# georgeyounes/CRIMP

Measured on AMD Instinct MI355X. Metric: Z^2_2 photon*trial evals/sec (node), higher is better.
Workload: dtype f64; 1 GPU; config3: synthetic 10000000 photons x 1000000 trials/GPU, Z^2_2; photons=10000000, trials_per_gpu=1000000, nharm=2, parallelism=trial-sharded dp1: sharding.sharded_search + all_gather(best), precision=default

## Files before the change

crimp_amd/csrc/search_nufft.h:

```cpp
#pragma once

typedef double nu_f64x4 __attribute__((ext_vector_type(4)));

constexpr int kNuCW = 1024;
constexpr int kNuWaves = 4;
constexpr int kNuRows = 8;
constexpr int kNuMaxP = 16;
constexpr int kNuGatherMaxP = 24;
constexpr int kNuMergeG = 16;
constexpr int kNuMaxWrap = 32;
constexpr int kNuTile = 4096;
constexpr double kNuEps = 5e-14;
constexpr double kNuEpsZm = 5e-13;
constexpr double kNuRho = 1e-13;

constexpr int kNuPassMax = 10;
struct NuPass {
    int64_t gmin[kNuPassMax];
    int64_t ubase[kNuPassMax];
};

struct NuTw {
    const double2* lo;
    const double2* hi;
// ... 429 lines not shown
        }
    }
    for (int o = L / 2; o > 0; o >>= 1)
#pragma unroll
        for (int r = 0; r < R; ++r)
#pragma unroll
            for (int p = 0; p < PP; ++p)
                if (p < P) {
                    ar[r][p] += __shfl_xor(ar[r][p], o);
                    ai[r][p] += __shfl_xor(ai[r][p], o);
                }
#pragma unroll
    for (int r = 0; r < R; ++r)
#pragma unroll
        for (int p = 0; p < PP; ++p)
            if (r < nrow && p < P && (p & (L - 1)) == sub)
                W[((int64_t)p * nrow + r) * nfft + g] = make_double2(ar[r][p], ai[r][p]);
}

__global__ __launch_bounds__(256) void k_nu_merge(const double* __restrict__ U, int64_t SL,
                                                  const int64_t* __restrict__ ctab, int64_t nchunk, int64_t gmin,
                                                  int64_t gmax, int64_t nfft, int64_t gbase, int64_t gcount,
                                                  double2* __restrict__ W, const int* __restrict__ bad) {
    if (*bad) return;
    __shared__ int64_t rs[kNuMergeG][kNuMaxWrap];
    __shared__ int rc[kNuMergeG][kNuMaxWrap];
    __shared__ int nr[kNuMergeG];
    extern __shared__ double nu_acc[];
    const int64_t i0 = (int64_t)blockIdx.x * kNuMergeG;
    const int tid = threadIdx.x;
    if (tid < kNuMergeG) {
        const int64_t g = (gbase + i0 + tid) & (nfft - 1);
        int cnt = 0;
        if (i0 + tid < gcount) {
            int64_t Gu = gmin + (((g - gmin) % nfft) + nfft) % nfft;
            for (; Gu <= gmax && cnt < kNuMaxWrap; Gu += nfft) {
                int64_t lo = 0, hi = nchunk;
                while (lo < hi) {
                    const int64_t mid = (lo + hi) >> 1;
                    if (ctab[2 * mid + 1] < Gu)
                        lo = mid + 1;
                    else
                        hi = mid;
                }
                int len = 0;
                while (lo + len < nchunk && ctab[2 * (lo + len)] <= Gu) ++len;
                if (len > 0) {
                    rs[tid][cnt] = Gu - gmin + lo;
                    rc[tid][cnt] = len;
                    ++cnt;
                }
            }
        }
        nr[tid] = cnt;
    }
    __syncthreads();
    for (int64_t idx = tid; idx < kNuMergeG * SL; idx += 256) {
        const int t = (int)(idx / SL);
        const int64_t e = idx - t * SL;
        double v = 0.0;
        for (int r = 0; r < nr[t]; ++r)
            for (int k = 0; k < rc[t][r]; ++k) v += U[(rs[t][r] + k) * SL + e];
        nu_acc[idx] = v;
    }
    __syncthreads();
    const int64_t B = SL / 2;
    for (int64_t idx = tid; idx < kNuMergeG * B; idx += 256) {
        const int t = (int)(idx % kNuMergeG);
        const int64_t beta = idx / kNuMergeG;
        if (i0 + t < gcount) {
            const int64_t g = (gbase + i0 + t) & (nfft - 1);
            W[beta * nfft + g] = make_double2(nu_acc[t * SL + 2 * beta], nu_acc[t * SL + 2 * beta + 1]);
        }
    }
}

__device__ __forceinline__ void nu_power(const double2* __restrict__ CS, int64_t nbt, int64_t t, int m, int stat,
                                         double nph, double E, bool lastv, double2 last, double* pout,
                                         double* eout) {
    const double w = 2.0 / nph;
    auto zk = [&](int k, double* amag) {
        const double2 a = (lastv && k == m - 1) ? last : CS[(int64_t)k * nbt + t];
        const double z = a.x * a.x + a.y * a.y;
        *amag = sqrt(z);
        return z;
    };
    double p, err;
    if (stat == CRIMP_STAT_Z2) {
        double zsum = 0.0, eb = 0.0, am;
        for (int k = 0; k < m; ++k) {
            zsum += zk(k, &am);
            eb += 2.0 * am * E + E * E;
        }
        p = zsum * w;
        err = eb * w;
    } else {
        double cum = 0.0, best = -INFINITY, ebest = 0.0, eacc = 0.0, am;
        for (int k = 0; k < m; ++k) {
            const double z = zk(k, &am);
            cum += z * w;
            eacc += (2.0 * am * E + E * E) * w;
            const double v = cum - 4.0 * (double)k;
            if (v > best) {
                best = v;
                ebest = eacc;
            }
        }
        p = best;
        err = ebest;
        cum = 0.0;
        eacc = 0.0;
        for (int k = 0; k < m; ++k) {
            const double z = zk(k, &am);
            cum += z * w;
            eacc += (2.0 * am * E + E * E) * w;
            if (cum - 4.0 * (double)k + eacc >= best - ebest) err = fmax(err, eacc);
        }
    }
    *pout = p;
    *eout = err;
}
__device__ __forceinline__ double nu_err_bound(int64_t jc, int64_t nfft, int P, double invfact, double nph) {
    const double x = 3.14159265358979323846 * fabs((double)jc) / (double)nfft;
    double xp = 1.0;
    for (int p = 0; p < P; ++p) xp *= x;
    return nph * (xp * invfact + kNuRho);
}

__device__ __forceinline__ void nu_dft2(double2* v) {
    const double2 a = v[0], b = v[1];
    v[0] = nu_add(a, b);
    v[1] = nu_sub(a, b);
}
__device__ __forceinline__ void nu_dft4(double2& a0, double2& a1, double2& a2, double2& a3) {
    const double2 t0 = nu_add(a0, a2), t1 = nu_sub(a0, a2), t2 = nu_add(a1, a3), t3 = nu_muli(nu_sub(a1, a3));
    a0 = nu_add(t0, t2);
    a2 = nu_sub(t0, t2);
    a1 = nu_add(t1, t3);
    a3 = nu_sub(t1, t3);
}
__device__ __forceinline__ void nu_dft4v(double2* v) { nu_dft4(v[0], v[1], v[2], v[3]); }
__device__ __forceinline__ void nu_dft8(double2* v) {
    double2 e[4] = {v[0], v[2], v[4], v[6]}, o[4] = {v[1], v[3], v[5], v[7]};
    nu_dft4v(e);
    nu_dft4v(o);
    const double s = 0.70710678118654752440084436210485;
    const double2 w[4] = {make_double2(1.0, 0.0), make_double2(s, s), make_double2(0.0, 1.0), make_double2(-s, s)};
#pragma unroll
    for (int k = 0; k < 4; ++k) {
        const double2 t = k == 0 ? o[0] : k == 2 ? nu_muli(o[2]) : nu_cmul(o[k], w[k]);
        v[k] = nu_add(e[k], t);
        v[k + 4] = nu_sub(e[k], t);
    }
}
__device__ __forceinline__ void nu_dft16(double2* v) {
    double2 e[8], o[8];
#pragma unroll
    for (int k = 0; k < 8; ++k) {
        e[k] = v[2 * k];
        o[k] = v[2 * k + 1];
    }
    nu_dft8(e);
    nu_dft8(o);
    const double c1 = 0.92387953251128675612818318939679, s1 = 0.38268343236508977172845998403040,
                 r2 = 0.70710678118654752440084436210485;
    const double2 w[8] = {make_double2(1.0, 0.0), make_double2(c1, s1), make_double2(r2, r2), make_double2(s1, c1),
                          make_double2(0.0, 1.0), make_double2(-s1, c1), make_double2(-r2, r2), make_double2(-c1, s1)};
#pragma unroll
    for (int k = 0; k < 8; ++k) {
        const double2 t = k == 0 ? o[0] : k == 4 ? nu_muli(o[4]) : nu_cmul(o[k], w[k]);
        v[k] = nu_add(e[k], t);
        v[k + 8] = nu_sub(e[k], t);
    }
}
template <int R>
__device__ __forceinline__ void nu_dft(double2* v) {
    if (R == 2) nu_dft2(v);
    else if (R == 4) nu_dft4v(v);
    else if (R == 8) nu_dft8(v);
    else nu_dft16(v);
}

struct NuTile {
    double2 hi[64], lo[64];
};
__device__ __forceinline__ void nu_tile_init(NuTile* tw, int lt) {
    const int t = threadIdx.x;
    if (t < 128) {
        const int m = t < 64 ? t : (t - 64) << 6;
        double sv, cv;
        sincospi(ldexp((double)m, 1 - lt), &sv, &cv);
        if (t < 64)
            tw->lo[t] = make_double2(cv, sv);
        else
            tw->hi[t - 64] = make_double2(cv, sv);
    }
}
__device__ __forceinline__ double2 nu_tw_tile(const NuTile* tw, int m) { return nu_cmul(tw->hi[m >> 6], tw->lo[m & 63]); }

template <int R>
__device__ __forceinline__ void nu_twiddle(double2 w, double2* v) {
    double2 b[4];
    b[0] = w;
#pragma unroll
    for (int i = 1; i < 4; ++i)
        if ((1 << i) < R) b[i] = nu_cmul(b[i - 1], b[i - 1]);
#pragma unroll
    for (int r = 1; r < R; ++r) {
        double2 wr = make_double2(1.0, 0.0);
        bool first = true;
#pragma unroll
        for (int i = 0; i < 4; ++i)
            if (r & (1 << i)) {
                wr = first ? b[i] : nu_cmul(wr, b[i]);
                first = false;
            }
        v[r] = nu_cmul(v[r], wr);
    }
}

template <int R>
__device__ __forceinline__ void nu_stage(double2* s, int ll, int lc, int sa, int sc, int lns, const NuTile* tw,
                                         int lt) {
    constexpr int NB = 16 / R;
    constexpr int LR = R == 2 ? 1 : R == 4 ? 2 : R == 8 ? 3 : 4;
    const int L = 1 << ll, Ns = 1 << lns;
    const int nbt = (L >> LR) << lc;
    double2 v[NB][R];
#pragma unroll
    for (int k = 0; k < NB; ++k) {
        const int b = threadIdx.x + 256 * k;
        if (b < nbt) {
            const int cc = b & ((1 << lc) - 1), j = b >> lc;
#pragma unroll
            for (int r = 0; r < R; ++r) v[k][r] = s[(j + (r << (ll - LR))) * sa + cc * sc];
            if (lns > 0) {
                nu_twiddle<R>(nu_tw_tile(tw, (j & (Ns - 1)) << (lt - lns - LR)), v[k]);
            }
            nu_dft<R>(v[k]);
        }
    }
    __syncthreads();
#pragma unroll
    for (int k = 0; k < NB; ++k) {
        const int b = threadIdx.x + 256 * k;
        if (b < nbt) {
            const int cc = b & ((1 << lc) - 1), j = b >> lc;
            const int base = ((j >> lns) << (lns + LR)) + (j & (Ns - 1));
#pragma unroll
            for (int r = 0; r < R; ++r) s[(base + r * Ns) * sa + cc * sc] = v[k][r];
        }
    }
    __syncthreads();
}

__device__ __forceinline__ void nu_fft_lds(double2* s, int ll, int lc, int sa, int sc, const NuTile* tw, int lt) {
    int lns = 0;
    while (lns < ll) {
        const int rem = ll - lns;
        if (rem >= 4) {
            nu_stage<16>(s, ll, lc, sa, sc, lns, tw, lt);
            lns += 4;
        } else if (rem == 3) {
            nu_stage<8>(s, ll, lc, sa, sc, lns, tw, lt);
            lns += 3;
        } else if (rem == 2) {
            nu_stage<4>(s, ll, lc, sa, sc, lns, tw, lt);
            lns += 2;
        } else {
            nu_stage<2>(s, ll, lc, sa, sc, lns, tw, lt);
            lns += 1;
        }
    }
}

__global__ __launch_bounds__(256) __attribute__((amdgpu_waves_per_eu(2))) void k_nu_fft_cols(const double2* __restrict__ X, double2* __restrict__ Y,
                                                     int lnfft, int ln1, int lc, NuTw T, int alo, int acnt) {
    extern __shared__ double2 nu_s[];
    __shared__ NuTile tw;
    const int lt = lnfft < 12 ? lnfft : 12;
    nu_tile_init(&tw, lt);
    const int ln2 = lnfft - ln1, c = 1 << lc, n1 = 1 << ln1;
    const int64_t nfft = int64_t(1) << lnfft;
    const int64_t b0 = (int64_t)blockIdx.x << lc;
    const double2* x = X + (int64_t)blockIdx.y * nfft;
    double2* y = Y + (int64_t)blockIdx.y * nfft;
    for (int e = threadIdx.x; e < (n1 << lc); e += 256) {
        const int a = e >> lc, cc = e & (c - 1);
        nu_s[e] = ((a - alo) & (n1 - 1)) < acnt ? x[((int64_t)a << ln2) + b0 + cc] : make_double2(0.0, 0.0);
    }
    __syncthreads();
    nu_fft_lds(nu_s, ln1, lc, c, 1, &tw, lt);
#pragma unroll
    for (int q = 0; q < kNuTile / 256; ++q) {
        const int e = threadIdx.x + 256 * q;
        if (e < (n1 << lc)) {
            const int k1 = e >> lc, cc = e & (c - 1);
            const int64_t b = b0 + cc;
            y[((int64_t)k1 << ln2) + b] = nu_cmul(nu_s[e], nu_tw(T, b * k1));
        }
    }
}

__global__ __launch_bounds__(256) __attribute__((amdgpu_waves_per_eu(2))) void k_nu_cols256(
    const double2* __restrict__ X, double2* __restrict__ Y, int lnfft, NuTw T, int alo, int acnt, int64_t ngroups) {
    extern __shared__ double2 nu_s[];
    __shared__ NuTile tw;
    nu_tile_init(&tw, 12);
    const int ln2 = lnfft - 8;
    const int64_t nfft = int64_t(1) << lnfft;
    const int cc = threadIdx.x & 15, j = threadIdx.x >> 4;
    const int64_t cpb = int64_t(1) << (ln2 - 4);
    double2 nv[16], tf[4];
    auto fetch = [&](int64_t grp) {
        const int64_t b = ((grp % cpb) << 4) + cc;
        const double2* x = X + (grp / cpb) * nfft + b;
        const int64_t lm = (int64_t(1) << T.lbits) - 1, tb = (b * (int64_t)j) & T.mask, ts = (b << 4) & T.mask;
        tf[0] = T.hi[tb >> T.lbits];
        tf[1] = T.lo[tb & lm];
        tf[2] = T.hi[ts >> T.lbits];
        tf[3] = T.lo[ts & lm];
#pragma unroll
        for (int r = 0; r < 16; ++r) {
            const int a = j + 16 * r;
            nv[r] = ((a - alo) & 255) < acnt ? x[(int64_t)a << ln2] : make_double2(0.0, 0.0);
        }
    };
    int64_t grp = blockIdx.x;
    if (grp < ngroups) fetch(grp);
    __syncthreads();
    for (; grp < ngroups; grp += gridDim.x) {
        double2 v[16];
#pragma unroll
        for (int r = 0; r < 16; ++r) v[r] = nv[r];
        const double2 wb = nu_cmul(tf[0], tf[1]), ws = nu_cmul(tf[2], tf[3]);
        const int64_t b = ((grp % cpb) << 4) + cc;
        double2* y = Y + (grp / cpb) * nfft + b;
        if (grp + gridDim.x < ngroups) fetch(grp + gridDim.x);
        nu_dft16(v);
#pragma unroll
        for (int r = 0; r < 16; ++r) nu_s[((j << 4) + r) * 16 + cc] = v[r];
        __syncthreads();
#pragma unroll
        for (int r = 0; r < 16; ++r) v[r] = nu_s[(j + 16 * r) * 16 + cc];
        __syncthreads();
        nu_twiddle<16>(nu_tw_tile(&tw, j << 4), v);
        nu_dft16(v);
        v[0] = nu_cmul(v[0], wb);
        nu_twiddle<16>(ws, v);
#pragma unroll
        for (int r = 1; r < 16; ++r) v[r] = nu_cmul(v[r], wb);
#pragma unroll
        for (int r = 0; r < 16; ++r) y[(int64_t)(j + 16 * r) << ln2] = v[r];
    }
}

__global__ __launch_bounds__(512) __attribute__((amdgpu_waves_per_eu(4))) void k_nu_cols512(
    const double2* __restrict__ X, double2* __restrict__ Y, int lnfft, NuTw T, int alo, int acnt, int64_t ngroups) {
    constexpr int NC = 1, C = 8;
    extern __shared__ double2 nu_s[];
    __shared__ NuTile tw;
    nu_tile_init(&tw, 9);
    const int ln2 = lnfft - 9;
    const int64_t nfft = int64_t(1) << lnfft;
    const int cc = threadIdx.x & 7, j = threadIdx.x >> 3;
    const int64_t cpb = int64_t(1) << (ln2 - 3);
    double2 nv[NC][8], tf[NC][4];
    const int voff = ((j << ln2) + cc) * 16;
    auto fetch = [&](int64_t grp) {
        const int64_t b0 = (grp % cpb) * C;
        const __amdgpu_buffer_rsrc_t rs = __builtin_amdgcn_make_buffer_rsrc(
            (void*)(X + (grp / cpb) * nfft + b0), (short)0, (int)(16 << lnfft), 0x00020000);
        const int64_t lm = (int64_t(1) << T.lbits) - 1;
#pragma unroll
        for (int c = 0; c < NC; ++c) {
            const int64_t b = b0 + cc + 8 * c, tb = (b * (int64_t)j) & T.mask, ts = (b << 6) & T.mask;
            tf[c][0] = T.hi[tb >> T.lbits];
            tf[c][1] = T.lo[tb & lm];
            tf[c][2] = T.hi[ts >> T.lbits];
            tf[c][3] = T.lo[ts & lm];
        }
#pragma unroll
        for (int q = 0; q < 8; ++q) {
            const bool occ = ((j + 64 * q - alo) & 511) < acnt;
#pragma unroll
            for (int c = 0; c < NC; ++c)
                nv[c][q] = occ ? __builtin_bit_cast(double2, __builtin_amdgcn_raw_buffer_load_b128(
                                                                 rs, voff, ((64 * q << ln2) + 8 * c) * 16, 0))
                               : make_double2(0.0, 0.0);
        }
    };
    int64_t grp = blockIdx.x;
    if (grp < ngroups) fetch(grp);
    const int m2 = (j & 7) << 3;
    const int z2 = ((j >> 3) << 6) + (j & 7);
    __syncthreads();
    typedef unsigned int nu_u4 __attribute__((ext_vector_type(4)));
    for (; grp < ngroups; grp += gridDim.x) {
        double2 v[NC][8], wb[NC], ws[NC];
#pragma unroll
        for (int c = 0; c < NC; ++c) {
#pragma unroll
            for (int q = 0; q < 8; ++q) v[c][q] = nv[c][q];
            wb[c] = nu_cmul(tf[c][0], tf[c][1]);
            ws[c] = nu_cmul(tf[c][2], tf[c][3]);
        }
        const __amdgpu_buffer_rsrc_t ry = __builtin_amdgcn_make_buffer_rsrc(
            (void*)(Y + (grp / cpb) * nfft + (grp % cpb) * C), (short)0, (int)(16 << lnfft), 0x00020000);
        if (grp + gridDim.x < ngroups) fetch(grp + gridDim.x);
#pragma unroll
        for (int c = 0; c < NC; ++c) {
            nu_dft8(v[c]);
#pragma unroll
            for (int q = 0; q < 8; ++q) nu_s[((j << 3) + q) * C + cc + 8 * c] = v[c][q];
        }
        __syncthreads();
#pragma unroll
        for (int c = 0; c < NC; ++c) {
#pragma unroll
            for (int q = 0; q < 8; ++q) v[c][q] = nu_s[(j + 64 * q) * C + cc + 8 * c];
        }
        __syncthreads();
        const double2 t2 = nu_tw_tile(&tw, m2);
#pragma unroll
        for (int c = 0; c < NC; ++c) {
            nu_twiddle<8>(t2, v[c]);
            nu_dft8(v[c]);
#pragma unroll
            for (int q = 0; q < 8; ++q) nu_s[(z2 + 8 * q) * C + cc + 8 * c] = v[c][q];
        }
        __syncthreads();
#pragma unroll
        for (int c = 0; c < NC; ++c) {
#pragma unroll
            for (int q = 0; q < 8; ++q) v[c][q] = nu_s[(j + 64 * q) * C + cc + 8 * c];
        }
        __syncthreads();
        const double2 t3 = nu_tw_tile(&tw, j);
#pragma unroll
        for (int c = 0; c < NC; ++c) {
            nu_twiddle<8>(t3, v[c]);
            nu_dft8(v[c]);
            v[c][0] = nu_cmul(v[c][0], wb[c]);
            nu_twiddle<8>(ws[c], v[c]);
#pragma unroll
            for (int q = 1; q < 8; ++q) v[c][q] = nu_cmul(v[c][q], wb[c]);
        }
#pragma unroll
        for (int q = 0; q < 8; ++q) {
#pragma unroll
            for (int c = 0; c < NC; ++c)
                __builtin_amdgcn_raw_buffer_store_b128(__builtin_bit_cast(nu_u4, v[c][q]), ry, voff,
                                                       ((64 * q << ln2) + 8 * c) * 16, 0);
        }
    }
}

constexpr int kNuFusedPer = kNuTile / 256;
__global__ __launch_bounds__(256) __attribute__((amdgpu_waves_per_eu(1))) void k_nu_fft_rows_combine(const double2* __restrict__ X, int ll, int lnfft, int P,
                                                             int nrow, int64_t nf, int64_t jhi, int64_t h,
                                                             int64_t tbase, int64_t nbt, const double* __restrict__ bc,
                                                             double2* __restrict__ CS) {
    extern __shared__ double2 nu_s[];
    __shared__ NuTile tw;
    const int lt = lnfft < 12 ? lnfft : 12;
    nu_tile_init(&tw, lt);
    const int64_t nfft = int64_t(1) << lnfft;
    const int L = 1 << ll, ln1 = lnfft - ll;
    const int64_t k1 = blockIdx.x;
    const int r = blockIdx.y;
    double2 acc[kNuFusedPer], nx[kNuFusedPer];
    NuBes bs[kNuFusedPer];
    const double2* xr = X + (int64_t)r * nfft + (k1 << ll);
    const int64_t pstride = (int64_t)nrow * nfft;
#pragma unroll
    for (int q = 0; q < kNuFusedPer; ++q) {
        acc[q] = make_double2(0.0, 0.0);
        const int e = threadIdx.x + 256 * q;
        const int64_t J = k1 + ((int64_t)e << ln1);
        bs[q] = nu_bes_start(bc, P, nu_zh(J <= jhi ? J : J - nfft, lnfft));
        nx[q] = e < L ? xr[(int64_t)(P - 1) * pstride + e] : make_double2(0.0, 0.0);
    }
    for (int p = P - 1; p >= 0; --p) {
        const int64_t pn = (int64_t)(p > 0 ? p - 1 : 0) * pstride;
#pragma unroll
        for (int q = 0; q < kNuFusedPer; ++q) {
            const int e = threadIdx.x + 256 * q;
            if (e < L) {
                nu_s[e] = nx[q];
                nx[q] = xr[pn + e];
            }
        }
        __syncthreads();
        nu_fft_lds(nu_s, ll, 0, 1, L, &tw, lt);
#pragma unroll
        for (int q = 0; q < kNuFusedPer; ++q) {
            const int b = threadIdx.x + 256 * q;
            if (b < L) {
                const double2 v = nu_s[b];
                const int64_t J = k1 + ((int64_t)b << ln1);
                const int64_t jc = J <= jhi ? J : J - nfft;
                acc[q] = nu_bes_acc(acc[q], nu_bes_w(bs[q], p, nu_zh(jc, lnfft)), v, p);
            }
        }
        __syncthreads();
    }
#pragma unroll
    for (int q = 0; q < kNuFusedPer; ++q) {
        const int b = threadIdx.x + 256 * q;
        if (b >= L) continue;
        const int64_t J = k1 + ((int64_t)b << ln1);
        int64_t jc;
        if (J <= jhi)
            jc = J;
        else if (J >= nfft - h)
            jc = J - nfft;
        else
            continue;
        const int64_t t = tbase + r * nf + jc;
        if (t >= 0 && t < nbt) CS[t] = acc[q];
    }
}

struct NuFinal {
    int on, m, stat, Pc;
    double nph, invfact, rel;
    int64_t tb0;
    double* out;
    int* nflag;
    int64_t* flagged;
    BestCand* best_part;
    int64_t best_base;
    const double2* CS0;
};
template <int TPB, int NP>
__device__ __forceinline__ void nu_rows_epilogue(const double2 (&acc)[NP], int64_t k1, int ln1, int64_t nfft,
                                                 int64_t jhi, int64_t h, int64_t tbase, int r, int64_t nf, int64_t nbt,
                                                 double2* __restrict__ CS, const NuFinal& F, double2* lds,
                                                 int pos0 = -1) {
    const int t = threadIdx.x;
    const int b0 = pos0 < 0 ? t : pos0;
    if (!F.on) {
#pragma unroll
        for (int q = 0; q < NP; ++q) {
            const int64_t J = k1 + ((int64_t)(b0 + TPB * q) << ln1);
            int64_t jc;
            if (J <= jhi)
                jc = J;
            else if (J >= nfft - h)
                jc = J - nfft;
            else
                continue;
            const int64_t tt = tbase + r * nf + jc;
            if (tt >= 0 && tt < nbt) CS[tt] = acc[q];
        }
        return;
    }
    BestCand bc_ = {-INFINITY, INT64_MAX};
#pragma unroll
    for (int q = 0; q < NP; ++q) {
        const int64_t J = k1 + ((int64_t)(b0 + TPB * q) << ln1);
        int64_t jc;
        if (J <= jhi)
            jc = J;
        else if (J >= nfft - h)
            jc = J - nfft;
        else
            continue;
        const int64_t tt = tbase + r * nf + jc;
        if (tt < 0 || tt >= nbt) continue;
        double p, err;
        nu_power(F.CS0, nbt, tt, F.m, F.stat, F.nph, nu_err_bound(jc, nfft, F.Pc, F.invfact, F.nph), true, acc[q], &p,
                 &err);
        F.out[F.tb0 + tt] = p;
        if (!(err <= F.rel * fabs(p))) F.flagged[atomicAdd(F.nflag, 1)] = F.tb0 + tt;
        if (best_better(p, F.tb0 + tt, bc_.v, bc_.i)) bc_ = {p, F.tb0 + tt};
    }
    if (!F.best_part) return;
    for (int o = 32; o > 0; o >>= 1) {
        const double v = __shfl_xor(bc_.v, o);
        const int64_t i = __shfl_xor(bc_.i, o);
        if (best_better(v, i, bc_.v, bc_.i)) bc_ = {v, i};
    }
    __syncthreads();
    BestCand* red = reinterpret_cast<BestCand*>(lds);
    if ((t & 63) == 0) red[t >> 6] = bc_;
    __syncthreads();
    if (t == 0) {
        for (int w = 1; w < TPB / 64; ++w)
            if (best_better(red[w].v, red[w].i, bc_.v, bc_.i)) bc_ = red[w];
        F.best_part[F.best_base + (int64_t)blockIdx.y * gridDim.x + blockIdx.x] = bc_;
    }
}

struct NuRot {
    double j1, j2, iz2;
};
constexpr size_t nu_rows_lds(int ln2) { return 2 * ((size_t(1) << ln2) + (size_t(1) << (ln2 - 3))) * sizeof(double2); }
template <int LN2>
__global__ __launch_bounds__(1 << (LN2 - 3)) __attribute__((amdgpu_waves_per_eu(2))) void k_nu_rows_combine8(
    const double2* X, int lnfft, int P, int plo, int accum, int nrow, int64_t nf, int64_t jhi, int64_t h,
    int64_t tbase, int64_t nbt, const double* __restrict__ bc, double2* __restrict__ CS, const NuFinal F) {
    constexpr int N = 1 << LN2, TPB = N / 8, NT = N + N / 8;
    constexpr int Ns2 = 4, Ns3 = 8 * Ns2;
    static_assert(LN2 == 11, "rows of 2048");
    extern __shared__ double2 nu_s[];
    __shared__ NuTile tw;
    nu_tile_init(&tw, LN2);
    const int64_t nfft = int64_t(1) << lnfft;
    const int ln1 = lnfft - LN2;
    const int64_t k1 = blockIdx.x;
    const int r = blockIdx.y;
    const int t = threadIdx.x;
    const double2* xr = X + (int64_t)r * nfft + (k1 << LN2);
    const int64_t pstride = (int64_t)nrow * nfft;
    auto load_row = [&](int pm, double2 (&dst)[8]) {
        const __amdgpu_buffer_rsrc_t rs =
            __builtin_amdgcn_make_buffer_rsrc((void*)(xr + (int64_t)pm * pstride), (short)0, N * 16, 0x00020000);
#pragma unroll
        for (int q = 0; q < 8; ++q)
            dst[q] = __builtin_bit_cast(double2, __builtin_amdgcn_raw_buffer_load_b128(rs, t * 16, TPB * 16 * q, 0));
    };
    double2 acc[8], xa[8], xb[8];
    NuRot bs[8];
    const int rP = P & 3;
#pragma unroll
    for (int q = 0; q < 8; ++q) {
        double2 a0 = make_double2(0.0, 0.0);
        const int64_t J = k1 + ((int64_t)(t + TPB * q) << ln1);
        const int64_t jc = J <= jhi ? J : J - nfft;
        if (accum) {
            const int64_t tt = tbase + r * nf + jc;
            if ((J <= jhi || J >= nfft - h) && tt >= 0 && tt < nbt) a0 = CS[tt];
        }
        acc[q] = rP == 0 ? a0 : rP == 1 ? make_double2(a0.y, -a0.x) : rP == 2 ? make_double2(-a0.x, -a0.y)
                                                                        : make_double2(-a0.y, a0.x);
        const NuBes b0 = nu_bes_start(bc, P, nu_zh(jc, lnfft));
        bs[q] = {2.0 * b0.j1, 2.0 * b0.j2, b0.iz2};
    }
    load_row(P - 1 - plo, xa);
    const int m2 = (t & (Ns2 - 1)) * (N / (8 * Ns2)), m3 = (t & (Ns3 - 1)) * (N / (8 * Ns3)), m4 = t;
    const int z2 = (t / Ns2) * 8 * Ns2 + (t & (Ns2 - 1)), z3 = (t / Ns3) * 8 * Ns3 + (t & (Ns3 - 1));
    const int w1 = 4 * t + (t >> 1), w2 = z2 + (z2 >> 3), w3 = z3 + (z3 >> 3), rd = t + (t >> 3);
    __syncthreads();
    auto moment = [&](auto LAST, int p, double2 (&v)[8], double2 (&nv)[8], double2* A, double2* B) {
        constexpr bool last = decltype(LAST)::value;
        if (p > plo) load_row(p - 1 - plo, nv);
        nu_dft4(v[0], v[2], v[4], v[6]);
        nu_dft4(v[1], v[3], v[5], v[7]);
#pragma unroll
        for (int q = 0; q < 4; ++q) {
            A[w1 + q] = v[2 * q];
            A[w1 + N / 2 + N / 16 + q] = v[2 * q + 1];
        }
        __syncthreads();
#pragma unroll
        for (int q = 0; q < 8; ++q) v[q] = A[rd + TPB * 9 / 8 * q];
        nu_twiddle<8>(nu_tw_tile(&tw, m2), v);
// ... 378 lines not shown
        if (!(std::fabs(a) < glim && std::fabs(b) < glim)) return false;
        pl->gmin[(size_t)(k - 1)] = (int64_t)std::rint(a);
        pl->gmax[(size_t)(k - 1)] = (int64_t)std::rint(b);
        if (pl->gmax[(size_t)(k - 1)] < pl->gmin[(size_t)(k - 1)]) return false;
        if ((pl->gmax[(size_t)(k - 1)] - pl->gmin[(size_t)(k - 1)]) / nfft + 1 > kNuMaxWrap) return false;
    }
    return true;
}

static bool nu_gather_form(int64_t nrows_grid) {
    const char* spread_env = getenv("CRIMP_NUFFT_SPREAD");
    return spread_env && !strcmp(spread_env, "gather")  ? true
           : spread_env && !strcmp(spread_env, "mfma") ? false
                                                       : nrows_grid <= kNuGatherRows;
}

struct NuSpecKey {
    const void* t;
    const void* f;
    int64_t n, nf, nfd, first, count;
    double t0;
    int nharm, stat, dev, gather;
    bool operator==(const NuSpecKey& o) const {
        return t == o.t && f == o.f && n == o.n && nf == o.nf && nfd == o.nfd && first == o.first &&
               count == o.count && t0 == o.t0 && nharm == o.nharm && stat == o.stat && dev == o.dev &&
               gather == o.gather;
    }
};
struct NuSpecEntry {
    NuSpecKey key;
    double hs[5];
};
static std::vector<NuSpecEntry> g_nu_spec;
static bool nu_spec_disabled() {
    const char* e = getenv("CRIMP_NUFFT_PLAN_CACHE");
    return e && !strcmp(e, "0");
}
static NuSpecKey nu_spec_key(const double* t, int64_t n, double t0, const double* f, int64_t nf, int64_t nfd,
                             int nharm, int stat, int64_t first, int64_t count, bool gather) {
    NuSpecKey k{};
    k.stat = stat;
    k.t = t;
    k.f = f;
    k.n = n;
    k.nf = nf;
    k.nfd = nfd;
    k.first = first;
    k.count = count;
    k.t0 = t0;
    k.nharm = nharm;
    k.gather = gather ? 1 : 0;
    (void)hipGetDevice(&k.dev);
    return k;
}
static bool nu_spec_find(const NuSpecKey& k, double* hs) {
    if (nu_spec_disabled()) return false;
    for (const NuSpecEntry& e : g_nu_spec)
        if (e.key == k) {
            std::memcpy(hs, e.hs, sizeof(e.hs));
            return true;
        }
    return false;
}
static void nu_spec_drop(const NuSpecKey& k) {
    for (size_t i = 0; i < g_nu_spec.size(); ++i)
        if (g_nu_spec[i].key == k) {
            g_nu_spec.erase(g_nu_spec.begin() + (std::ptrdiff_t)i);
            return;
        }
}
static void nu_spec_store(const NuSpecKey& k, const double* hs) {
    if (nu_spec_disabled()) return;
    nu_spec_drop(k);
    if (g_nu_spec.size() >= 16) g_nu_spec.erase(g_nu_spec.begin());
    NuSpecEntry e;
    e.key = k;
    std::memcpy(e.hs, hs, sizeof(e.hs));
    g_nu_spec.push_back(e);
}

static bool nu_row_groups(std::vector<NuPlan>* plans, int64_t first, int64_t count, int64_t nf, double delta, double f0,
                          double dt0, double dtn, int nharm, int pmax, double eps) {
    const int64_t r_lo = first / nf, r_hi = (first + count - 1) / nf;
    for (int64_t r = r_lo; r <= r_hi;) {
        const int64_t a = std::max<int64_t>(first, r * nf) - r * nf, b = std::min<int64_t>(first + count, (r + 1) * nf) - r * nf;
        int64_t r1 = r + 1;
        if (a == 0 && b == nf)
            while (r1 <= r_hi && std::min<int64_t>(first + count, (r1 + 1) * nf) - r1 * nf == nf) ++r1;
        NuPlan pl;
        pl.r0 = r;
        pl.r1 = r1;
        pl.j0 = a;
        pl.nseg = b - a;
        if (pl.nseg < 64 || !nu_plan(&pl, delta, f0, dt0, dtn, nharm + 1, pmax, eps)) return false;
        plans->push_back(std::move(pl));
        r = r1;
    }
    return true;
}

static int64_t nu_spread_passes(std::vector<std::pair<int, int>>* passes, const std::vector<NuPlan>& plans, int nharm,
                                int64_t nchunk, int64_t fixed_bytes) {
    int64_t ubytes = 0;
    for (int Gmax = 10;; Gmax = Gmax == 10 ? 8 : Gmax / 2) {
        passes->clear();
        ubytes = 0;
        for (int k0 = 1; k0 <= nharm;) {
            const int rem = nharm - k0 + 1;
            int gl = 2;
            for (int cand : {10, 8, 6, 4, 2})
                if (cand <= Gmax && cand <= rem + 1) {
                    gl = cand;
                    break;
                }
            for (const NuPlan& pl : plans) {
                const int64_t SLmax = 2 * (int64_t)pl.P * std::min<int64_t>(kNuRows, pl.r1 - pl.r0);
                int64_t sl = 0;
                for (int k = k0; k < k0 + gl; ++k)
                    sl += (pl.gmax[(size_t)(k - 1)] - pl.gmin[(size_t)(k - 1)] + 1 + nchunk) * SLmax;
                ubytes = std::max<int64_t>(ubytes, sl * 8);
            }
            passes->emplace_back(k0, gl);
            k0 += gl;
        }
        if (Gmax == 2 || ubytes + fixed_bytes <= nufft_budget()) break;
    }
    return ubytes;
}

static bool nu_generic_fft() {
    const char* e = getenv("CRIMP_NUFFT_ROWS4096");
    return e && !strcmp(e, "0");
}

static int nu_rows_lds_attrs() {
    static std::mutex mu;
    static uint64_t done = 0;
    int dev = 0;
    HIPCHK(hipGetDevice(&dev));
    std::lock_guard<std::mutex> lk(mu);
    if (dev >= 64 || !(done >> dev & 1)) {
        HIPCHK(hipFuncSetAttribute(reinterpret_cast<const void*>(k_nu_rows_iw),
                                   hipFuncAttributeMaxDynamicSharedMemorySize, 2 * kNuTile * (int)sizeof(double2)));
        HIPCHK(hipFuncSetAttribute(reinterpret_cast<const void*>(k_nu_rows_combine8<11>),
                                   hipFuncAttributeMaxDynamicSharedMemorySize, (int)nu_rows_lds(11)));
        if (dev < 64) done |= uint64_t(1) << dev;
    }
    return CRIMP_OK;
}

static int nufft_search(Scratch& sc, hipStream_t s, const double* t, double t0, int64_t n, const double* freq,
                        int64_t nf, int64_t nrows_grid, const double* c2, const double* hs, bool twod, int nharm,
                        int stat, int64_t first,
                        int64_t count, double* out, bool timed, int64_t* nfixed, bool no_fixup, bool* applicable,
                        double* best, bool* best_done, int* nflag, bool* mismatch) {
    *applicable = false;
    *best_done = false;
    *nfixed = 0;
    *mismatch = false;
    int bad = 0;
    memcpy(&bad, hs + 4, sizeof(int));
    if (bad) return CRIMP_OK;
    const double delta = hs[0], f0 = hs[1], dt0 = hs[2], dtn = hs[3];
    const int64_t nchunk = cdiv(n, kNuCW);
    const bool gather_grid = nu_gather_form(nrows_grid);
    std::vector<NuPlan> plans;
    if (!nu_row_groups(&plans, first, count, nf, delta, f0, dt0, dtn, nharm, gather_grid ? kNuGatherMaxP : kNuMaxP,
                       stat == 0 && nharm >= 2 ? kNuEpsZm : kNuEps))
        return CRIMP_OK;
    *applicable = true;
    g_last_search_path = 2;
    g_last_nufft_n = 0;
    for (const NuPlan& pl : plans)
        if ((int64_t(1) << pl.lnfft) > g_last_nufft_n) {
            g_last_nufft_n = int64_t(1) << pl.lnfft;
            g_last_nufft_p = pl.P;
        }
    g_last_nufft_gather = gather_grid ? 1 : 0;
    for (double& w : g_nu_work) w = 0.0;
    int64_t Bmax = 0, nfmax = 0, csmax = 0, nrow_all = 0;
    for (const NuPlan& pl : plans) {
        const int64_t nrow_max = std::min<int64_t>(kNuRows, pl.r1 - pl.r0);
        const int lrow = 12 - std::min(pl.lnfft, 12);
        Bmax = std::max<int64_t>(Bmax, (cdiv((int64_t)pl.P * nrow_max, int64_t(1) << lrow) << lrow) << pl.lnfft);
        csmax = std::max<int64_t>(csmax, (int64_t)nharm * nrow_max * pl.nseg);
        nfmax = std::max<int64_t>(nfmax, int64_t(1) << pl.lnfft);
        nrow_all = std::max<int64_t>(nrow_all, nrow_max);
    }
    int gw = 1;
    if (gather_grid) {
        gw = std::min(nharm, kNuGatherSet);
        while (gw > 1 && (gw + 1) * Bmax * 16 + csmax * 16 > nufft_budget()) --gw;
    }
    const int64_t fixed_bytes = (gw + 1) * Bmax * 16 + csmax * 16;
    std::vector<std::pair<int, int>> passes;
    const int64_t ubytes = nu_spread_passes(&passes, plans, nharm, nchunk, fixed_bytes);
    const bool generic_fft = nu_generic_fft();
    {
        const int rc = nu_rows_lds_attrs();
        if (rc) return rc;
    }
    const char* lanes_s = getenv("CRIMP_NUFFT_LANES");
    const int lanes_env = lanes_s ? atoi(lanes_s) : 0;
    ARGCHK(lanes_env == 0 || lanes_env == 1 || lanes_env == 2 || lanes_env == 4 || lanes_env == 8,
           "CRIMP_NUFFT_LANES must be 1, 2, 4 or 8");
    int64_t starts_max = 0;
    if (gather_grid)
        for (const NuPlan& pl : plans) {
            int64_t tot = 0;
            for (int k = 1; k <= nharm; ++k) tot += pl.gmax[(size_t)(k - 1)] - pl.gmin[(size_t)(k - 1)] + 2;
            starts_max = std::max<int64_t>(starts_max, tot);
        }
    double* U = nullptr;
    double2 *W = nullptr, *Y = nullptr, *CS = nullptr;
    int64_t* ctab = nullptr;
    int64_t* cstart = nullptr;
    int64_t* flagged = nullptr;
    if (!gather_grid) {
        HIPCHK(sc.alloc(&U, (size_t)(ubytes / 8)));
        HIPCHK(sc.alloc(&ctab, (size_t)(2 * kNuPassMax * nchunk)));
    }
    if (starts_max > 0) HIPCHK(sc.alloc(&cstart, (size_t)starts_max));
    HIPCHK(sc.alloc(&W, (size_t)(Bmax * gw)));
    HIPCHK(sc.alloc(&Y, (size_t)Bmax));
    HIPCHK(sc.alloc(&CS, (size_t)csmax));
    HIPCHK(sc.alloc(&flagged, (size_t)count));
    BestCand* best_part = nullptr;
    int64_t best_count = 0, separate_batches = 0;
    if (best) {
        int64_t nb = 0;
        for (const NuPlan& pl : plans) nb += (pl.r1 - pl.r0) * (int64_t(1) << (pl.lnfft - std::min(pl.lnfft, 12)));
        HIPCHK(sc.alloc(&best_part, (size_t)std::max<int64_t>(nb, 1)));
    }
    std::vector<NuPass> hps;
    for (const NuPlan& pl : plans) {
        for (int64_t rb = pl.r0; !gather_grid && rb < pl.r1; rb += kNuRows) {
            const int64_t SL = 2 * (int64_t)pl.P * std::min<int64_t>(kNuRows, pl.r1 - rb);
            for (const auto& pass : passes) {
                NuPass ps{};
                int64_t off = 0;
                for (int kk = 0; kk < pass.second; ++kk) {
                    const int k = pass.first + kk;
                    ps.gmin[kk] = pl.gmin[(size_t)(k - 1)];
                    ps.ubase[kk] = off;
                    off += (pl.gmax[(size_t)(k - 1)] - pl.gmin[(size_t)(k - 1)] + 1 + nchunk) * SL;
                }
                hps.push_back(ps);
            }
        }
    }
    NuPass* dps = nullptr;
    if (!hps.empty()) {
        HIPCHK(sc.alloc(&dps, hps.size()));
        HIPCHK(hipMemcpyAsync(dps, hps.data(), hps.size() * sizeof(NuPass), hipMemcpyHostToDevice, s));
    }
    size_t ipass = 0;
    const size_t lds_fft = (size_t)kNuTile * sizeof(double2);
    std::vector<hipEvent_t> ev;
    std::vector<int> evcls;
    auto mark = [&]() -> hipError_t {
        if (!timed) return hipSuccess;
        hipEvent_t e = nullptr;
        hipError_t r = hipEventCreate(&e);
        if (r != hipSuccess) return r;
        ev.push_back(e);
        return hipEventRecord(e, s);
    };
    auto span = [&](int cls) -> hipError_t {
        if (!timed) return hipSuccess;
        evcls.push_back(cls);
        return mark();
    };
    int cur_lnfft = -1;
    NuTw T{};
    const double2* cis = nullptr;
    const double2* cis2 = nullptr;
    const double* bc = nullptr;
    for (const NuPlan& pl : plans) {
        if (pl.lnfft != cur_lnfft) {
            const int rc = nu_tables(sc, s, pl.lnfft, &T, &cis, &bc, &cis2);
            if (rc) return rc;
            cur_lnfft = pl.lnfft;
        }
        if (ev.empty()) HIPCHK(mark());
        const int lnfft = pl.lnfft, P = pl.P;
        const int64_t nfft = int64_t(1) << lnfft;
        const int ln2 = std::min(lnfft, 12), ln1 = lnfft - ln2;
        const int lcol = 12 - ln1;
        const int64_t jbase = pl.j0 + pl.h;
        auto occupied = [&](int k, int* alo, int* acnt) {
            nu_occupied(pl.gmin[(size_t)(k - 1)], pl.gmax[(size_t)(k - 1)], lnfft, ln1, alo, acnt);
        };
        const bool fuse_final = ln2 >= 11 && !generic_fft && !nu_final_separate();
        bool final_done = false;
        auto fft_combine = [&](int k, int64_t rb, int nrow, int64_t tb0, int64_t nbt, const double2* W) -> int {
            const int64_t Bp = (int64_t)P * nrow;
            const double plane = 16.0 * (double)Bp * (double)nfft;
            const double2* Z = W;
            if (ln1 > 0) {
                int alo = 0, acnt = 0;
                occupied(k, &alo, &acnt);
                g_nu_work[kNuClsPass1] += plane * ((double)acnt / (double)(int64_t(1) << ln1)) + plane;
                if (ln1 == 8 && !generic_fft) {
                    const int64_t ngroups = Bp << (ln2 - 4);
                    k_nu_cols256<<<(unsigned)std::min<int64_t>(ngroups, 2 * nu_cus()), 256, lds_fft, s>>>(
                        W, Y, lnfft, T, alo, acnt, ngroups);
                } else if (ln1 == 9 && !generic_fft) {
                    const int64_t ngroups = Bp << (ln2 - 3);
                    k_nu_cols512<<<(unsigned)std::min<int64_t>(ngroups, 2 * nu_cus()), 512, lds_fft, s>>>(
                        W, Y, lnfft, T, alo, acnt, ngroups);
                } else {
                    k_nu_fft_cols<<<dim3((unsigned)(int64_t(1) << (ln2 - lcol)), (unsigned)Bp), 256, lds_fft, s>>>(
                        W, Y, lnfft, ln1, lcol, T, alo, acnt);
                }
                HIPCHK(hipGetLastError());
                Z = Y;
                HIPCHK(span(kNuClsPass1));
            }
            NuFinal F{};
            if (fuse_final && k == nharm) {
                F.on = 1;
                F.m = nharm;
                F.stat = stat;
                F.Pc = P;
                F.nph = (double)n;
                F.invfact = pl.invfact;
                F.rel = fixup_rel();
                F.tb0 = tb0;
                F.out = out;
                F.nflag = nflag;
                F.flagged = flagged;
                F.best_part = best ? best_part : nullptr;
                F.best_base = best_count;
                F.CS0 = CS;
                best_count += (int64_t(1) << ln1) * nrow;
                final_done = true;
            }
            g_nu_work[kNuClsPass2] += plane + (F.on ? (16.0 * (nharm - 1) + 8.0) * (double)nbt : 16.0 * (double)nbt);
            const dim3 g2((unsigned)(int64_t(1) << ln1), (unsigned)nrow);
            const int64_t jhi = pl.nseg - 1 - pl.h, tbase = rb * nf + jbase - (tb0 + first);
            double2* CSk = CS + (int64_t)(k - 1) * nbt;
            if (ln2 == 12 && !generic_fft)
                k_nu_rows_iw<<<g2, 512, 2 * lds_fft, s>>>(Z, lnfft, P, 0, 0, nrow, nf, jhi, pl.h, tbase, nbt, bc, CSk, F);
            else if (ln2 == 11 && !generic_fft)
                k_nu_rows_combine8<11><<<g2, 256, nu_rows_lds(11), s>>>(Z, lnfft, P, 0, 0, nrow, nf, jhi, pl.h, tbase, nbt,
                                                                         bc, CSk, F);
            else
                k_nu_fft_rows_combine<<<g2, 256, lds_fft, s>>>(Z, ln2, lnfft, P, nrow, nf, jhi, pl.h, tbase, nbt, bc, CSk);
            HIPCHK(hipGetLastError());
            HIPCHK(span(kNuClsPass2));
            return CRIMP_OK;
        };
        auto finalize =[&](int64_t tb0, int64_t nbt) -> int {
            g_nu_work[kNuClsFinalize] += 16.0 * (double)nharm * (double)nbt + 8.0 * (double)nbt;
            k_nu_finalize<<<(unsigned)cdiv(nbt, 256), 256, 0, s>>>(CS, nbt, nharm, stat, (double)n, nf, jbase, nfft, P,
                                                                   pl.invfact, fixup_rel(), tb0, first, out, nflag,
                                                                   flagged);
            HIPCHK(hipGetLastError());
            HIPCHK(span(kNuClsFinalize));
            return CRIMP_OK;
        };
        if (gather_grid) {
            std::vector<int64_t> soff((size_t)nharm);
            int64_t off = 0;
            for (int k0 = 1; k0 <= nharm; k0 += kNuCellK) {
                NuCellArgs ca{};
                const int nk = std::min(kNuCellK, nharm - k0 + 1);
                for (int j = 0; j < nk; ++j) {
                    const int k = k0 + j;
                    ca.gmin[j] = pl.gmin[(size_t)(k - 1)];
                    ca.span[j] = pl.gmax[(size_t)(k - 1)] - pl.gmin[(size_t)(k - 1)] + 1;
                    ca.off[j] = off;
                    soff[(size_t)(k - 1)] = off;
                    off += ca.span[j] + 1;
                }
                const unsigned cb = (unsigned)std::min<int64_t>(cdiv(cdiv(n, 2), 256 * kNuCellU), 2048);
                if ((reinterpret_cast<uintptr_t>(t) & 15u) == 0)
                    k_nu_cellstart<true><<<cb, 256, 0, s>>>(t, t0, n, pl.s1, k0, nk, ca, cstart, nflag + 1);
                else
                    k_nu_cellstart<false><<<cb, 256, 0, s>>>(t, t0, n, pl.s1, k0, nk, ca, cstart, nflag + 1);
                HIPCHK(hipGetLastError());
            }
            HIPCHK(span(kNuClsCellStart));
            for (int64_t rb = pl.r0; rb < pl.r1; rb += kNuGatherRows) {
                const int nrow = (int)std::min<int64_t>(kNuGatherRows, pl.r1 - rb);
                const int64_t tb0 = std::max<int64_t>(first, rb * nf) - first;
                const int64_t nbt = std::min<int64_t>(first + count, (rb + nrow) * nf) - first - tb0;
                for (int k0 = 1; k0 <= nharm; k0 += gw) {
                    NuGatherSet S{};
                    S.nk = std::min(gw, nharm - k0 + 1);
                    int64_t blocks = 0, set_cells = 0;
                    for (int jj = 0; jj < S.nk; ++jj) {
                        int alo = 0, acnt = 0;
                        occupied(k0 + jj, &alo, &acnt);
                        set_cells += (int64_t)acnt << ln2;
                    }
                    for (int jj = 0; jj < S.nk; ++jj) {
                        const int k = k0 + jj;
                        int alo = 0, acnt = 0;
                        occupied(k, &alo, &acnt);
                        const int64_t gbase = (int64_t)alo << ln2, gcount = (int64_t)acnt << ln2;
                        const int64_t kspan = pl.gmax[(size_t)(k - 1)] - pl.gmin[(size_t)(k - 1)] + 1;
                        const int64_t ppc = n / std::max<int64_t>(1, std::min<int64_t>(kspan, nfft));
                        int L = 1;
                        while (L < 4 && set_cells * 2 * L <= (int64_t(1) << 20) && ppc >= 4 * 2 * L) L *= 2;
                        if (lanes_env > 0) L = lanes_env;
                        S.k[jj] = k;
                        S.lanes_log2[jj] = L == 8 ? 3 : L == 4 ? 2 : L == 2 ? 1 : 0;
                        S.blk0[jj] = blocks;
                        blocks += cdiv(gcount * L, 256);
                        S.gmin[jj] = pl.gmin[(size_t)(k - 1)];
                        S.gmax[jj] = pl.gmax[(size_t)(k - 1)];
                        S.gbase[jj] = gbase;
                        S.gcount[jj] = gcount;
                        S.soff[jj] = soff[(size_t)(k - 1)];
                        S.woff[jj] = (int64_t)jj * Bmax;
                        g_nu_work[0] += (40.0 + 5.0 * P) * (double)n * nrow;
                        g_nu_work[kNuClsSpread] += 8.0 * (double)n + 16.0 * (double)P * nrow * (double)gcount;
                    }
                    S.blk0[S.nk] = blocks;
                    launch_gather(twod, blocks, t, t0, cstart, nfft, pl.s1, pl.fch, pl.fcl, twod ? c2 + rb : nullptr,
                                  nrow, P, S, nflag + 1, cis2, W, s);
                    HIPCHK(hipGetLastError());
                    HIPCHK(span(kNuClsSpread));
                    for (int jj = 0; jj < S.nk; ++jj) {
                        int rc = fft_combine(k0 + jj, rb, nrow, tb0, nbt, W + (int64_t)jj * Bmax);
                        if (rc) return rc;
                    }
                }
                if (final_done) {
                    final_done = false;
                    continue;
                }
                ++separate_batches;
                int rc = finalize(tb0, nbt);
                if (rc) return rc;
            }
            continue;
        }
        for (int64_t rb = pl.r0; rb < pl.r1; rb += kNuRows) {
            const int nrow = (int)std::min<int64_t>(kNuRows, pl.r1 - rb);
            const int64_t tb0 = std::max<int64_t>(first, rb * nf) - first;
            const int64_t tb1 = std::min<int64_t>(first + count, (rb + nrow) * nf) - first;
            const int64_t nbt = tb1 - tb0;
            const int64_t SL = 2 * (int64_t)P * nrow;
            for (const auto& pass : passes) {
                const int k0 = pass.first, gl = pass.second;
                const NuPass& ps = hps[ipass];
                const NuPass* dp = dps + ipass++;
                dim3 grid((unsigned)cdiv(nchunk, kNuWaves));
                g_nu_work[0] += 512.0 * (double)n * gl;
                g_nu_work[kNuClsSpread] += 8.0 * (double)n;
                for (int kk = 0; kk < gl; ++kk)
                    g_nu_work[kNuClsSpread] += 8.0 * (double)SL *
                                    (double)(pl.gmax[(size_t)(k0 + kk - 1)] - ps.gmin[kk] + 1 + nchunk);
                if (twod)
                    nu_launch_spread<true>(gl, grid, s, t, t0, n, nchunk, pl.s1, pl.fch, pl.fcl, c2 + rb, nrow, k0, P, dp, cis,
                                           U, ctab, nflag + 1);
                else
                    nu_launch_spread<false>(gl, grid, s, t, t0, n, nchunk, pl.s1, pl.fch, pl.fcl, c2 + rb, nrow, k0, P, dp,
                                            cis, U, ctab, nflag + 1);
                HIPCHK(hipGetLastError());
                HIPCHK(span(kNuClsSpread));
                for (int kk = 0; kk < gl && k0 + kk <= nharm; ++kk) {
                    const int k = k0 + kk;
                    int alo = 0, acnt = 0;
                    occupied(k, &alo, &acnt);
                    const int64_t gbase = (int64_t)alo << ln2, gcount = (int64_t)acnt << ln2;
                    g_nu_work[kNuClsMerge] += 8.0 * (double)SL * (double)(pl.gmax[(size_t)(k - 1)] - ps.gmin[kk] + 1 + nchunk) +
                                    16.0 * (double)P * nrow * (double)gcount;
                    k_nu_merge<<<(unsigned)cdiv(gcount, kNuMergeG), 256, (size_t)kNuMergeG * SL * sizeof(double), s>>>(
                        U + ps.ubase[kk], SL, ctab + 2 * kk * nchunk, nchunk, ps.gmin[kk], pl.gmax[(size_t)(k - 1)],
                        nfft, gbase, gcount, W, nflag + 1);
                    HIPCHK(hipGetLastError());
                    HIPCHK(span(kNuClsMerge));
                    int rc = fft_combine(k, rb, nrow, tb0, nbt, W);
                    if (rc) return rc;
                }
            }
            if (final_done) {
                final_done = false;
                continue;
            }
            ++separate_batches;
            int rc = finalize(tb0, nbt);
            if (rc) return rc;
        }
    }
    if (timed) {
        HIPCHK(hipEventSynchronize(ev.back()));
        float tot = 0.0f;
        double cls[kNuCls] = {0, 0, 0, 0, 0, 0, 0}, cnt[kNuCls] = {0, 0, 0, 0, 0, 0, 0};
        HIPCHK(hipEventElapsedTime(&tot, ev.front(), ev.back()));
        for (size_t i = 1; i < ev.size(); ++i) {
            float ms = 0.0f;
            HIPCHK(hipEventElapsedTime(&ms, ev[i - 1], ev[i]));
            cls[evcls[i - 1]] += ms;
            cnt[evcls[i - 1]] += 1.0;
        }
        cnt[kNuClsCellStart] *= (nharm + kNuCellK - 1) / kNuCellK;
        for (hipEvent_t e : ev) (void)hipEventDestroy(e);
        if (g_kernel_times.empty()) g_last_kernel_ms = tot;
        g_kernel_times.push_back(tot);
        for (double v : cls) g_kernel_times.push_back(v);
        for (double v : cnt) g_kernel_times.push_back(v);
    }
    if (best) {
        if (separate_batches == 0 && best_count > 0) {
            k_best_final<<<1, 256, 0, s>>>(best_part, (int)best_count, reinterpret_cast<double*>(nflag + 4));
            HIPCHK(hipGetLastError());
        } else {
            const int rc = launch_best(sc, s, out, count, reinterpret_cast<double*>(nflag + 4));
            if (rc) return rc;
        }
    }
    int fl[8] = {0, 0, 0, 0, 0, 0, 0, 0};
    HIPCHK(d2h(s, fl, nflag, (best ? 8 : 2) * sizeof(int)));
    if (fl[1]) {
        *applicable = false;
        *mismatch = fl[1] == 2;
        g_last_search_path = 0;
        return CRIMP_OK;
    }
    const int nf_h = fl[0];
    *nfixed = nf_h;
    if (best && (nf_h == 0 || no_fixup)) {
        std::memcpy(best, fl + 4, 2 * sizeof(double));
        *best_done = true;
    }
    if (nf_h == 0 || no_fixup) return CRIMP_OK;
    double *dt = nullptr, *dt2 = nullptr;
    HIPCHK(sc.alloc(&dt, (size_t)n));
    if (twod) HIPCHK(sc.alloc(&dt2, (size_t)n));
    k_search_prep<<<(int)std::min<int64_t>(cdiv(n, 256), 4096), 256, 0, s>>>(t, n, t0, dt, dt2);
    HIPCHK(hipGetLastError());
    return fixup_search(sc, s, dt, dt2, n, freq, nf, c2, twod, nharm, stat, first, flagged, nf_h, out);
}
```

Baseline: 24610000 billion equivalent photon*trial evals/s.

## Restructure 256-point column FFT kernel into per-wave groups with wave-local transpose

Rewrites k_nu_cols256 so that each wavefront handles its own group of 4 columns instead of the whole block sharing 16 columns. The inter-stage transpose now goes through small per-wave padded LDS tiles, synchronised with wave barriers rather than block-wide __syncthreads, and real and imaginary parts are exchanged separately. Loads and stores use raw buffer intrinsics, the register double-buffered prefetch is dropped, and occupancy is raised to 4 waves per EU with no dynamic LDS. The change removes block barriers and LDS pressure, but it gives up the prefetch overlap and makes each column access narrower. It also leaves several compile-time variants selected by a macro.

```diff
diff --git a/crimp_amd/csrc/search_nufft.h b/crimp_amd/csrc/search_nufft.h
--- a/crimp_amd/csrc/search_nufft.h
+++ b/crimp_amd/csrc/search_nufft.h
@@ -755,58 +755,174 @@
     }
 }
 
-__global__ __launch_bounds__(256) __attribute__((amdgpu_waves_per_eu(2))) void k_nu_cols256(
+constexpr int kNuXe = 4 * 17;
+__device__ __forceinline__ void nu_wave_sync() {
+    __builtin_amdgcn_fence(__ATOMIC_RELEASE, "wavefront");
+    __builtin_amdgcn_wave_barrier();
+    __builtin_amdgcn_fence(__ATOMIC_ACQUIRE, "wavefront");
+}
+#ifndef NU_C256
+#define NU_C256 0
+#endif
+#if NU_C256 == 5
+__global__ __launch_bounds__(256) __attribute__((amdgpu_waves_per_eu(4, 4))) void k_nu_cols256(
     const double2* __restrict__ X, double2* __restrict__ Y, int lnfft, NuTw T, int alo, int acnt, int64_t ngroups) {
     extern __shared__ double2 nu_s[];
+    double* const ts = reinterpret_cast<double*>(nu_s);
     __shared__ NuTile tw;
     nu_tile_init(&tw, 12);
     const int ln2 = lnfft - 8;
     const int64_t nfft = int64_t(1) << lnfft;
-    const int cc = threadIdx.x & 15, j = threadIdx.x >> 4;
     const int64_t cpb = int64_t(1) << (ln2 - 4);
-    double2 nv[16], tf[4];
-    auto fetch = [&](int64_t grp) {
-        const int64_t b = ((grp % cpb) << 4) + cc;
-        const double2* x = X + (grp / cpb) * nfft + b;
-        const int64_t lm = (int64_t(1) << T.lbits) - 1, tb = (b * (int64_t)j) & T.mask, ts = (b << 4) & T.mask;
-        tf[0] = T.hi[tb >> T.lbits];
-        tf[1] = T.lo[tb & lm];
-        tf[2] = T.hi[ts >> T.lbits];
-        tf[3] = T.lo[ts & lm];
+    int tx = threadIdx.x;
+    typedef unsigned int nu_u4 __attribute__((ext_vector_type(4)));
+    __syncthreads();
+    for (int64_t grp = blockIdx.x; grp < ngroups; grp += gridDim.x) {
+        asm volatile("" : "+v"(tx));
+        const int cc = tx & 15, cj = tx >> 4;
+        const int b0 = (int)(grp % cpb) << 4;
+        const int64_t base = (grp / cpb) * nfft + b0;
+        const __amdgpu_buffer_rsrc_t rx =
+            __builtin_amdgcn_make_buffer_rsrc((void*)(X + base), (short)0, (int)(16 << lnfft), 0x00020000);
+        const __amdgpu_buffer_rsrc_t ry =
+            __builtin_amdgcn_make_buffer_rsrc((void*)(Y + base), (short)0, (int)(16 << lnfft), 0x00020000);
+        const int voff = ((cj << ln2) + cc) * 16;
+        double2 v[16], u[16];
 #pragma unroll
         for (int r = 0; r < 16; ++r) {
-            const int a = j + 16 * r;
-            nv[r] = ((a - alo) & 255) < acnt ? x[(int64_t)a << ln2] : make_double2(0.0, 0.0);
-        }
-    };
-    int64_t grp = blockIdx.x;
-    if (grp < ngroups) fetch(grp);
+            const bool occ = ((cj + 16 * r - alo) & 255) < acnt;
+            v[r] = occ ? __builtin_bit_cast(double2, __builtin_amdgcn_raw_buffer_load_b128(rx, voff, (16 * r << ln2) * 16, 0))
+                       : make_double2(0.0, 0.0);
+        }
+        nu_dft16(v);
+#pragma unroll
+        for (int r = 0; r < 16; ++r) asm volatile("" : "+v"(v[r].x), "+v"(v[r].y));
+#pragma unroll
+        for (int h = 0; h < 2; ++h) {
+#pragma unroll
+            for (int r = 0; r < 16; ++r) ts[((cj << 4) + r) * 16 + cc] = h ? v[r].y : v[r].x;
+            __syncthreads();
+#pragma unroll
+            for (int r = 0; r < 16; ++r) {
+                const double x = ts[(cj + 16 * r) * 16 + cc];
+                if (h)
+                    u[r].y = x;
+                else
+                    u[r].x = x;
+            }
+            __syncthreads();
+        }
+        nu_twiddle<16>(nu_tw_tile(&tw, cj << 4), u);
+        nu_dft16(u);
+        const int b = b0 + cc, lm = (1 << T.lbits) - 1, tb = (b * cj) & (int)T.mask, tsh = (b << 4) & (int)T.mask;
+        const double2 wb = nu_cmul(T.hi[tb >> T.lbits], T.lo[tb & lm]);
+        const double2 ws = nu_cmul(T.hi[tsh >> T.lbits], T.lo[tsh & lm]);
+        u[0] = nu_cmul(u[0], wb);
+        nu_twiddle<16>(ws, u);
+#pragma unroll
+        for (int r = 1; r < 16; ++r) u[r] = nu_cmul(u[r], wb);
+#pragma unroll
+        for (int r = 0; r < 16; ++r)
+            __builtin_amdgcn_raw_buffer_store_b128(__builtin_bit_cast(nu_u4, u[r]), ry, voff, (16 * r << ln2) * 16, 0);
+    }
+}
+#else
+__global__ __launch_bounds__(256) __attribute__((amdgpu_waves_per_eu(4, 4))) void k_nu_cols256(
+    const double2* __restrict__ X, double2* __restrict__ Y, int lnfft, NuTw T, int alo, int acnt, int64_t ngroups) {
+#if NU_C256 == 2
+    __shared__ double xs[4 * 64 * 17];
+#else
+    __shared__ double xs[4 * 4 * kNuXe];
+#endif
+    __shared__ NuTile tw;
+    nu_tile_init(&tw, 12);
+    const int ln2 = lnfft - 8;
+    const int64_t nfft = int64_t(1) << lnfft;
+    const int64_t cpb = int64_t(1) << (ln2 - 2);
+    int tx = threadIdx.x;
+    const int wv = __builtin_amdgcn_readfirstlane(tx >> 6);
+#if NU_C256 == 2
+    double* const xw = xs + wv * (64 * 17);
+#else
+    double* const xw = xs + wv * (4 * kNuXe);
+#endif
+    typedef unsigned int nu_u4 __attribute__((ext_vector_type(4)));
     __syncthreads();
-    for (; grp < ngroups; grp += gridDim.x) {
-        double2 v[16];
-#pragma unroll
-        for (int r = 0; r < 16; ++r) v[r] = nv[r];
-        const double2 wb = nu_cmul(tf[0], tf[1]), ws = nu_cmul(tf[2], tf[3]);
-        const int64_t b = ((grp % cpb) << 4) + cc;
-        double2* y = Y + (grp / cpb) * nfft + b;
-        if (grp + gridDim.x < ngroups) fetch(grp + gridDim.x);
+    for (int64_t grp = (int64_t)blockIdx.x * 4 + wv; grp < ngroups; grp += (int64_t)gridDim.x * 4) {
+        asm volatile("" : "+v"(tx));
+        const int lane = tx & 63, cj = lane & 15, c4 = lane >> 4;
+        const int b0 = (int)(grp % cpb) << 2;
+        const int64_t base = (grp / cpb) * nfft + b0;
+        const __amdgpu_buffer_rsrc_t rx =
+            __builtin_amdgcn_make_buffer_rsrc((void*)(X + base), (short)0, (int)(16 << lnfft), 0x00020000);
+        const __amdgpu_buffer_rsrc_t ry =
+            __builtin_amdgcn_make_buffer_rsrc((void*)(Y + base), (short)0, (int)(16 << lnfft), 0x00020000);
+        const int voff = ((cj << ln2) + c4) * 16;
+        double2 v[16], u[16];
+#pragma unroll
+        for (int r = 0; r < 16; ++r) {
+            const bool occ = ((cj + 16 * r - alo) & 255) < acnt;
+            v[r] = occ ? __builtin_bit_cast(double2, __builtin_amdgcn_raw_buffer_load_b128(rx, voff, (16 * r << ln2) * 16, 0))
+                       : make_double2(0.0, 0.0);
+        }
         nu_dft16(v);
 #pragma unroll
-        for (int r = 0; r < 16; ++r) nu_s[((j << 4) + r) * 16 + cc] = v[r];
-        __syncthreads();
-#pragma unroll
-        for (int r = 0; r < 16; ++r) v[r] = nu_s[(j + 16 * r) * 16 + cc];
-        __syncthreads();
-        nu_twiddle<16>(nu_tw_tile(&tw, j << 4), v);
-        nu_dft16(v);
-        v[0] = nu_cmul(v[0], wb);
-        nu_twiddle<16>(ws, v);
-#pragma unroll
-        for (int r = 1; r < 16; ++r) v[r] = nu_cmul(v[r], wb);
-#pragma unroll
-        for (int r = 0; r < 16; ++r) y[(int64_t)(j + 16 * r) << ln2] = v[r];
-    }
-}
+        for (int r = 0; r < 16; ++r) asm volatile("" : "+v"(v[r].x), "+v"(v[r].y));
+#if NU_C256 == 3
+        for (int r = 0; r < 16; ++r) u[r] = v[r];
+#elif NU_C256 == 2
+#pragma unroll
+        for (int h = 0; h < 2; ++h) {
+#pragma unroll
+            for (int r = 0; r < 16; ++r) xw[(c4 * 16 + r) * 17 + cj] = h ? v[r].y : v[r].x;
+            nu_wave_sync();
+#pragma unroll
+            for (int r = 0; r < 16; ++r) {
+                const double x = xw[(c4 * 16 + cj) * 17 + r];
+                if (h)
+                    u[r].y = x;
+                else
+                    u[r].x = x;
+            }
+            nu_wave_sync();
+        }
+#else
+#pragma unroll
+        for (int h = 0; h < 2; ++h)
+#pragma unroll
+            for (int q = 0; q < 4; ++q) {
+                if ((cj >> 2) == q) {
+                    double* dst = xw + (cj & 3) * kNuXe + c4 * 17;
+#pragma unroll
+                    for (int r = 0; r < 16; ++r) dst[r] = h ? v[r].y : v[r].x;
+                }
+                nu_wave_sync();
+#pragma unroll
+                for (int e = 0; e < 4; ++e) {
+                    const double x = xw[e * kNuXe + c4 * 17 + cj];
+                    if (h)
+                        u[4 * q + e].y = x;
+                    else
+                        u[4 * q + e].x = x;
+                }
+                nu_wave_sync();
+            }
+#endif
+        nu_twiddle<16>(nu_tw_tile(&tw, cj << 4), u);
+        nu_dft16(u);
+        const int b = b0 + c4, lm = (1 << T.lbits) - 1, tb = (b * cj) & (int)T.mask, ts = (b << 4) & (int)T.mask;
+        const double2 wb = nu_cmul(T.hi[tb >> T.lbits], T.lo[tb & lm]);
+        const double2 ws = nu_cmul(T.hi[ts >> T.lbits], T.lo[ts & lm]);
+        u[0] = nu_cmul(u[0], wb);
+        nu_twiddle<16>(ws, u);
+#pragma unroll
+        for (int r = 1; r < 16; ++r) u[r] = nu_cmul(u[r], wb);
+#pragma unroll
+        for (int r = 0; r < 16; ++r)
+            __builtin_amdgcn_raw_buffer_store_b128(__builtin_bit_cast(nu_u4, u[r]), ry, voff, (16 * r << ln2) * 16, 0);
+    }
+}
+#endif
 
 __global__ __launch_bounds__(512) __attribute__((amdgpu_waves_per_eu(4))) void k_nu_cols512(
     const double2* __restrict__ X, double2* __restrict__ Y, int lnfft, NuTw T, int alo, int acnt, int64_t ngroups) {
@@ -1791,9 +1907,15 @@
                 occupied(k, &alo, &acnt);
                 g_nu_work[kNuClsPass1] += plane * ((double)acnt / (double)(int64_t(1) << ln1)) + plane;
                 if (ln1 == 8 && !generic_fft) {
+#if NU_C256 == 5
                     const int64_t ngroups = Bp << (ln2 - 4);
-                    k_nu_cols256<<<(unsigned)std::min<int64_t>(ngroups, 2 * nu_cus()), 256, lds_fft, s>>>(
+                    k_nu_cols256<<<(unsigned)std::min<int64_t>(ngroups, 4 * nu_cus()), 256, lds_fft / 2, s>>>(
                         W, Y, lnfft, T, alo, acnt, ngroups);
+#else
+                    const int64_t ngroups = Bp << (ln2 - 2);
+                    k_nu_cols256<<<(unsigned)std::min<int64_t>(cdiv(ngroups, 4), 4 * nu_cus()), 256, 0, s>>>(
+                        W, Y, lnfft, T, alo, acnt, ngroups);
+#endif
                 } else if (ln1 == 9 && !generic_fft) {
                     const int64_t ngroups = Bp << (ln2 - 3);
                     k_nu_cols512<<<(unsigned)std::min<int64_t>(ngroups, 2 * nu_cus()), 512, lds_fft, s>>>(
```

Measured after the change: 21970000 billion equivalent photon*trial evals/s. 0.893x the previous value.
